# YJxyzxyz/road-vision-system

Hardware: AMD Instinct MI355X
Metric: end-to-end frames/sec @1080p (preproc+YOLOv8n+SORT), 1/2/4/8 MI355X (higher is better)
Workload: dtype bf16

## Files before the change

road-vision-system_amd/csrc/conv.hip:

```cpp
#include <algorithm>
#include <cstdlib>
#include <cstring>
#include "conv.h"
#include "conv_common.h"

namespace rv {

template <int MR, int NR, int WC>
__global__ __launch_bounds__(256, 2) void conv_mfma_kernel(ConvArgs a) {
  constexpr int WP = 4 / WC;
  const int tid = threadIdx.x;
  const int wave = tid >> 6, lane = tid & 63;
  const int col = lane & 15, quad = lane >> 4;
  const int wp = wave % WP, wc = wave / WP;
  const int cout_pad = (a.Cout + 15) & ~15;
  const int cout0 = (blockIdx.y * WC + wc) * (16 * MR);
  const int HWo = a.Ho * a.Wo;
  const int M = a.B * HWo;
  const int pix0 = (blockIdx.x * WP + wp) * (16 * NR);
  if (cout0 >= cout_pad || pix0 >= M) return;

  const int cin_pad = (a.Cin + 31) & ~31;
  const int kspt = cin_pad >> 5;
  const int Kp = a.k * a.k * cin_pad;
// ... 107 lines not shown
          float* o = (float*)outp;
          const float4 pk = make_float4(v[0], v[1], v[2], v[3]);
          if (!up) {
            *(float4*)(o + opix * cs_ + co_) = pk;
          } else {
            for (int dy = 0; dy < 2; ++dy)
              for (int dx = 0; dx < 2; ++dx) {
                const size_t q = ((size_t)(b * 2 * a.Ho + 2 * oy + dy) * (2 * a.Wo) + 2 * ox + dx);
                *(float4*)(o + q * cs_ + co_) = pk;
              }
          }
        } else {
          uint16_t* o = (uint16_t*)outp;
          const uint2 pk = make_uint2(pack_bf16x2(v[0], v[1]), pack_bf16x2(v[2], v[3]));
          if (!up) {
            *(uint2*)(o + opix * cs_ + co_) = pk;
          } else {
            for (int dy = 0; dy < 2; ++dy)
              for (int dx = 0; dx < 2; ++dx) {
                const size_t q = ((size_t)(b * 2 * a.Ho + 2 * oy + dy) * (2 * a.Wo) + 2 * ox + dx);
                *(uint2*)(o + q * cs_ + co_) = pk;
              }
          }
        }
      }
    }
  }
}

template <int MR, int NR, int WC>
static void launch_t(const ConvArgs& a, hipStream_t s) {
  constexpr int WP = 4 / WC;
  const int M = a.B * a.Ho * a.Wo;
  const int T = (a.Cout + 15) / 16;
  dim3 grid(ceil_div(M, 16 * NR * WP), ceil_div(T, MR * WC));
  conv_mfma_kernel<MR, NR, WC><<<grid, 256, 0, s>>>(a);
}

static int try_launch_patch(const ConvArgs& a, hipStream_t s, int* st);

static bool vcat(const ConvArgs& a) { return a.split > 0 || a.in_up; }

int launch_conv(const ConvArgs& a, hipStream_t s) {
  int st = 0;
  if (vcat(a)) {
    const int T = (a.Cout + 15) / 16;
    ConvCfg c{1, 1, 1, 1, 1, 1};
    for (const int mr : {8, 4, 2})
      if (T % mr == 0 && conv_cfg_ok(a, ConvCfg{mr, 1, 1, 1, 1, 1})) {
        c.mr = mr;
        break;
      }
    if (!conv_cfg_ok(a, c)) {
      set_error("virtual concat input (split %d, up %d) needs a bf16 1x1 conv", a.split, a.in_up);
      return RV_EINVAL;
    }
    return launch_conv_cfg(a, c, s);
  }
  if (try_launch_patch(a, s, &st)) return st;
  if (a.ch_w) {
    set_error("chained 1x1 conv (Cout %d, k%d s%d) has no patch-kernel configuration", a.Cout, a.k,
              a.stride);
    return RV_EINVAL;
  }
  if (a.in8) {
    set_error("fp8 conv (Cin %d, Cout %d, k%d s%d) has no patch-kernel configuration", a.Cin,
              a.Cout, a.k, a.stride);
    return RV_EINVAL;
  }
  if (a.g2_cout0 > 0) {
    set_error("grouped conv (Cout %d, split %d) has no patch-kernel configuration", a.Cout,
              a.g2_cout0);
    return RV_EINVAL;
  }
  const int T = (a.Cout + 15) / 16;
  const long M = (long)a.B * a.Ho * a.Wo;
  struct Cand {
    int mr, nr;
  };
  static const Cand cands[] = {{4, 4}, {2, 8}, {4, 2}, {2, 4}, {1, 8}, {4, 1}, {2, 2},
                               {1, 4}, {2, 1}, {1, 2}, {1, 1}};
  int MR = 1, NR = 1;
  for (const Cand& c : cands) {
    if (c.mr > T) continue;
    const int waste = ceil_div(T, c.mr) * c.mr - T;
    if (waste > 1 && c.mr > 1) continue;
    const long waves = (long)ceil_div((int)((M + 16 * c.nr - 1) / (16 * c.nr)), 1) * ceil_div(T, c.mr);
    MR = c.mr;
    NR = c.nr;
    if (waves >= 2048) break;
  }
  const int groups_c = ceil_div(T, MR);
  const int WC = groups_c >= 4 ? 4 : (groups_c >= 2 ? 2 : 1);
#define RV_CONV_WC(mr, nr)                                           \
  if (MR == mr && NR == nr) {                                        \
    if (WC == 4) launch_t<mr, nr, 4>(a, s);                          \
    else if (WC == 2) launch_t<mr, nr, 2>(a, s);                     \
    else launch_t<mr, nr, 1>(a, s);                                  \
    return launch_status("conv_mfma");                               \
  }
  RV_CONV_WC(4, 4) RV_CONV_WC(2, 8) RV_CONV_WC(4, 2) RV_CONV_WC(2, 4) RV_CONV_WC(1, 8)
  RV_CONV_WC(4, 1) RV_CONV_WC(2, 2) RV_CONV_WC(1, 4) RV_CONV_WC(2, 1) RV_CONV_WC(1, 2)
  RV_CONV_WC(1, 1)
#undef RV_CONV_WC
  set_error("no conv variant for MR=%d NR=%d", MR, NR);
  return RV_EINVAL;
}

__device__ __attribute__((aligned(64))) uint4 g_zero16[4];
#ifdef RV_PHASE_PROF
__device__ unsigned long long g_conv_phase[8];
#define RV_PH_T() __builtin_amdgcn_s_memtime()
#endif

struct TileWalk {
  int t0, step, end;
  __device__ __forceinline__ int count() const { return t0 < end ? (end - t0 + step - 1) / step : 0; }
};
__device__ __forceinline__ TileWalk tile_walk(int ntiles) {
  const int gx = gridDim.x, bx = blockIdx.x;
  if ((gx & 7) == 0) {
    const int chunk = (ntiles + 7) >> 3, j = bx & 7;
    return TileWalk{j * chunk + (bx >> 3), gx >> 3, min(ntiles, (j + 1) * chunk)};
  }
  return TileWalk{bx, gx, ntiles};
}
static inline int xcd_grid(int want, int ntiles, bool persist) {
  if (!persist) return ntiles >= 8 ? (ntiles + 7) & ~7 : ntiles;
  const int g = std::min(want, ntiles);
  return g >= 8 ? g & ~7 : g;
}

#ifndef RV_CONV_IN_AUX
#define RV_CONV_IN_AUX 0
#endif
template <int AUX = 0>
__device__ __forceinline__ void dma16(__amdgpu_buffer_rsrc_t r, void* lds, uint32_t voff, int soff) {
  __builtin_amdgcn_raw_ptr_buffer_load_lds(r, (__attribute__((address_space(3))) void*)lds, 16,
                                           (int)voff, soff, 0, AUX);
}

__device__ __forceinline__ float head_sigmoid(float x) {
  return __builtin_amdgcn_rcpf(1.0f + __expf(-x));
}

struct PatchGeo {
  int C, R;
  int G;
  int PH, PW;
  int pinst;
  int tiles_x, tiles_y;
  int p_bytes;
  int fast;
  int stagger;
};

static bool epi_fast(const ConvArgs& a) {
  static const bool off = getenv("RV_EPI_SLOW") != nullptr;
  const double px = (double)a.B * a.Ho * a.Wo;
  return !off && !a.out_f32 && !a.out1 && !a.out0_up && !a.in8 && a.Cout % 16 == 0 && px < (1 << 23) &&
         a.out0_cs < 2048 && px * a.out0_cs * 2 < 2147483647.0 &&
         (!a.res || (a.res_cs < 2048 && px * a.res_cs * 2 < 2147483647.0));
}

template <int MR, int NR>
__device__ __forceinline__ void epilogue_fast(const ConvArgs& a, f32x4 (&acc)[MR][NR], int cout0,
                                              const bool (&pv)[NR], const uint32_t (&opx)[NR],
                                              int quad, const f32x4 (&bias)[MR]) {
  const __amdgpu_buffer_rsrc_t ro = __builtin_amdgcn_make_buffer_rsrc(a.out0, 0, 0x7FFFFFFF, kRsrcFlags);
  const __amdgpu_buffer_rsrc_t rr =
      __builtin_amdgcn_make_buffer_rsrc((void*)a.res, 0, 0x7FFFFFFF, kRsrcFlags);
  const int cq = cout0 + quad * 4;
  constexpr uint32_t kDrop = 0x80000000u;
  auto value = [&](int m, int n, uint32_t vr, uint32_t& lo, uint32_t& hi) {
    float v[4];
#pragma unroll
    for (int i = 0; i < 4; ++i) v[i] = acc[m][n][i] + bias[m][i];
    if (a.act) {
      silu4(v);
    }
    if (a.res) {
      const uint32_t roff = cout0 + m * 16 < a.Cout ? vr + m * 32 : kDrop;
      const uint2 q = __builtin_bit_cast(
          uint2, __builtin_amdgcn_raw_buffer_load_b64(rr, (int)roff, 0, 0));
      v[0] += bf2f(q.x & 0xFFFF);
      v[1] += bf2f(q.x >> 16);
      v[2] += bf2f(q.y & 0xFFFF);
      v[3] += bf2f(q.y >> 16);
    }
    lo = pack_bf16x2(v[0], v[1]);
    hi = pack_bf16x2(v[2], v[3]);
  };
#pragma unroll
  for (int n = 0; n < NR; ++n) {
    if (!pv[n]) continue;
    const uint32_t vo = (__umul24(opx[n], (uint32_t)a.out0_cs) + a.out0_co + cq) * 2;
    const uint32_t vr = a.res ? (__umul24(opx[n], (uint32_t)a.res_cs) + a.res_co + cq) * 2 : 0u;
    const uint32_t vo16 = vo + (16 * (quad & 1) + 8 * (quad >> 1) - 4 * quad) * 2;
#pragma unroll
    for (int m = 0; m + 1 < MR; m += 2) {
      if (cout0 + m * 16 >= a.Cout) continue;
      uint32_t a0, a1, b0, b1;
      value(m, n, vr, a0, a1);
      value(m + 1, n, vr, b0, b1);
      const auto x0 = __builtin_amdgcn_permlane16_swap(a0, b0, false, false);
      const auto x1 = __builtin_amdgcn_permlane16_swap(a1, b1, false, false);
      const bool ok = cout0 + (m + (quad & 1)) * 16 < a.Cout;
      const uint32_t off = ok ? vo16 + m * 32 : kDrop;
      const v4u32 pk = {x0[0], x1[0], x0[1], x1[1]};
      __builtin_amdgcn_raw_buffer_store_b128(pk, ro, (int)off, 0, 0);
    }
    if constexpr (MR & 1) {
      constexpr int m = MR - 1;
      if (cout0 + m * 16 < a.Cout) {
        uint32_t lo, hi;
        value(m, n, vr, lo, hi);
        __builtin_amdgcn_raw_buffer_store_b64(v2u32{lo, hi}, ro, (int)(vo + m * 32), 0, 0);
      }
    }
  }
}

template <int MR, int NR>
struct EpiPend {
  v4u32 pk[MR / 2 > 0 ? MR / 2 : 1][NR];
  uint32_t off[MR / 2 > 0 ? MR / 2 : 1][NR];
  v2u32 pk1[NR];
  uint32_t off1[NR];
};

template <int MR, int NR>
__device__ __forceinline__ void epi_pack(const ConvArgs& a, f32x4 (&acc)[MR][NR], int cout0,
                                         const bool (&pv)[NR], const uint32_t (&opx)[NR], int quad,
                                         const f32x4 (&bias)[MR], EpiPend<MR, NR>& ep) {
  const __amdgpu_buffer_rsrc_t rr =
      __builtin_amdgcn_make_buffer_rsrc((void*)a.res, 0, 0x7FFFFFFF, kRsrcFlags);
  const int cq = cout0 + quad * 4;
  constexpr uint32_t kDrop = 0x80000000u;
  uint2 rq[MR][NR];
  if (a.res) {
#pragma unroll
    for (int n = 0; n < NR; ++n) {
      const uint32_t vr = (__umul24(opx[n], (uint32_t)a.res_cs) + a.res_co + cq) * 2;
#pragma unroll
      for (int m = 0; m < MR; ++m) {
        const uint32_t roff = pv[n] && cout0 + m * 16 < a.Cout ? vr + m * 32 : kDrop;
        rq[m][n] = __builtin_bit_cast(uint2, __builtin_amdgcn_raw_buffer_load_b64(rr, (int)roff, 0, 0));
      }
    }
  }
  auto value = [&](int m, int n, uint32_t vr, uint32_t& lo, uint32_t& hi) {
    (void)vr;
    float v[4];
#pragma unroll
    for (int i = 0; i < 4; ++i) v[i] = acc[m][n][i] + bias[m][i];
    if (a.act) silu4(v);
    if (a.res) {
      const uint2 q = rq[m][n];
      v[0] += bf2f(q.x & 0xFFFF);
      v[1] += bf2f(q.x >> 16);
      v[2] += bf2f(q.y & 0xFFFF);
      v[3] += bf2f(q.y >> 16);
    }
    lo = pack_bf16x2(v[0], v[1]);
    hi = pack_bf16x2(v[2], v[3]);
  };
#pragma unroll
  for (int n = 0; n < NR; ++n) {
    const uint32_t vo = (__umul24(opx[n], (uint32_t)a.out0_cs) + a.out0_co + cq) * 2;
    const uint32_t vr = a.res ? (__umul24(opx[n], (uint32_t)a.res_cs) + a.res_co + cq) * 2 : 0u;
    const uint32_t vo16 = vo + (16 * (quad & 1) + 8 * (quad >> 1) - 4 * quad) * 2;
#pragma unroll
    for (int m = 0; m + 1 < MR; m += 2) {
      uint32_t a0, a1, b0, b1;
      value(m, n, vr, a0, a1);
      value(m + 1, n, vr, b0, b1);
      const auto x0 = __builtin_amdgcn_permlane16_swap(a0, b0, false, false);
      const auto x1 = __builtin_amdgcn_permlane16_swap(a1, b1, false, false);
      const bool ok = pv[n] && cout0 + (m + (quad & 1)) * 16 < a.Cout;
      ep.off[m / 2][n] = ok ? vo16 + m * 32 : kDrop;
      ep.pk[m / 2][n] = v4u32{x0[0], x1[0], x0[1], x1[1]};
    }
    if constexpr (MR & 1) {
      constexpr int m = MR - 1;
      uint32_t lo, hi;
      value(m, n, vr, lo, hi);
      ep.off1[n] = pv[n] && cout0 + m * 16 < a.Cout ? vo + m * 32 : kDrop;
      ep.pk1[n] = v2u32{lo, hi};
    }
  }
}

template <int MR, int NR>
__device__ __forceinline__ void epi_store(const ConvArgs& a, const EpiPend<MR, NR>& ep) {
  const __amdgpu_buffer_rsrc_t ro = __builtin_amdgcn_make_buffer_rsrc(a.out0, 0, 0x7FFFFFFF, kRsrcFlags);
#pragma unroll
  for (int n = 0; n < NR; ++n) {
#pragma unroll
    for (int m = 0; m + 1 < MR; m += 2)
      __builtin_amdgcn_raw_buffer_store_b128(ep.pk[m / 2][n], ro, (int)ep.off[m / 2][n], 0, 0);
    if constexpr (MR & 1) __builtin_amdgcn_raw_buffer_store_b64(ep.pk1[n], ro, (int)ep.off1[n], 0, 0);
  }
}

template <bool F8>
__device__ __forceinline__ int swzq(int i) {
  return F8 ? (i >> 2) & 3 : (i >> 1) & 2;
// ... 186 lines not shown
  bool oin[NR];
#pragma unroll
  for (int n = 0; n < NR; ++n) {
    const int q = wave * (NR * 16) + n * 16 + col;
    orow[n] = q / g.C;
    ocol[n] = q - orow[n] * g.C;
    oin[n] = q < g.R * g.C;
    const int pr = oin[n] ? orow[n] * S : 0, pc = oin[n] ? ocol[n] * S : 0;
#pragma unroll
    for (int kx = 0; kx < K; ++kx) {
      const int sc = patch_scol<S>(pc + kx, g.PW);
      const int lq = F8 ? quad >> 1 : quad;
      if constexpr (F8 && K == 3)
        boff[n][kx] = (pr * g.PW + sc) * 64 + swzq<true>(sc);
      else
        boff[n][kx] = (pr * g.PW + sc) * 64 + ((lq ^ swzq<F8>(sc)) << 4) + (F8 ? (quad & 1) * 8 : 0);
    }
  }
  int aoff[F8 && K == 3 ? MR : 1][2];
  if constexpr (F8 && K == 3) {
#pragma unroll
    for (int m = 0; m < MR; ++m) {
      const int row = m * 16 + col, sw = swzq<true>(row);
      const int base = (row * T2 + (quad >> 1)) * 64;
      aoff[m][0] = base + (((2 * (quad & 1)) ^ sw) << 4);
      aoff[m][1] = base + (((2 * (quad & 1) + 1) ^ sw) << 4);
    }
  }
  float* const bias_lds = (float*)(stages + 2 * stage_bytes);
  f32x4 bias[F8 ? MR : 1], dq[F8 ? MR : 1];
  if constexpr (F8) {
#pragma unroll
    for (int m = 0; m < MR; ++m) {
      const int co = wc0 + m * 16 + quad * 4;
      bias[m] = co < wcout_pad ? *(const f32x4*)(bias_p + co) : f32x4{0.f, 0.f, 0.f, 0.f};
      const f32x4 ws = co < wcout_pad ? *(const f32x4*)(wsc_p + co) : f32x4{0.f, 0.f, 0.f, 0.f};
      dq[m] = ws * a.s_in;
    }
  } else {
    for (int i = tid; i < BC; i += 64 * NW) bias_lds[i] = wc0 + i < wcout_pad ? bias_p[wc0 + i] : 0.f;
  }
  auto bias_tile = [&](f32x4 (&bl)[MR]) {
#pragma unroll
    for (int m = 0; m < MR; ++m) bl[m] = *(const f32x4*)(bias_lds + m * 16 + quad * 4);
  };
  constexpr int CHN = (MR + 1) / 2;
  constexpr int CHF = BC + 4;
  uint8_t* const ch_w_lds = (uint8_t*)(bias_lds + BC);
  float* const ch_b_lds = (float*)(ch_w_lds + (CH ? CHN * BC * 64 : 0));
  uint8_t* const ch_x_lds = (uint8_t*)(ch_b_lds + (CH ? BC : 0)) + wave * (CH ? CHN * NR * 16 * 64 : 0);
  float* const ch_f_lds = (float*)((uint8_t*)(ch_b_lds + (CH ? BC : 0)) + NW * (CH ? CHN * NR * 16 * 64 : 0)) +
                          wave * (CHM == 2 ? NR * 16 * CHF : 0);
  if constexpr (CH) {
    static_assert(!F8 && K == 3, "chained 1x1: bf16 behind a 3x3 conv");
    for (int j = wave; j < CHN * (BC / 16); j += NW) {
      const int c = j / (BC / 16), jr = j - c * (BC / 16);
      const int row = jr * 16 + (lane >> 2);
      const int q = (lane & 3) ^ swzq<false>(row);
      __builtin_amdgcn_global_load_lds((const void*)(a.ch_w + (size_t)row * (CHN * 32) + c * 32 + q * 8),
                                       (void*)(ch_w_lds + c * BC * 64 + jr * 1024), 16, 0, 0);
    }
    for (int i = tid; i < BC; i += 64 * NW) ch_b_lds[i] = a.ch_b[i];
    if constexpr (MR % 2) {
      for (int px = lane; px < NR * 16; px += 64) {
        uint8_t* sl = ch_x_lds + ((CHN - 1) * NR * 16 + px) * 64;
        *(uint4*)(sl + ((2 ^ swzq<false>(px)) << 4)) = make_uint4(0, 0, 0, 0);
        *(uint4*)(sl + ((3 ^ swzq<false>(px)) << 4)) = make_uint4(0, 0, 0, 0);
      }
    }
  }
  uint32_t tailbad = 0;
  int lgeo[MAXP];
#pragma unroll
  for (int it = 0; it < MAXP; ++it) {
    const int L = 64 * (wave + NW * it) + lane;
    const int pix = L / SL, q = L - SL * pix;
    const int py = (int)(((float)pix + 0.5f) * inv_pw);
    const int sc = pix - py * g.PW;
    const int he = (g.PW + 1) >> 1;
    const int px = S == 1 ? sc : (sc < he ? 2 * sc : 2 * (sc - he) + 1);
    const int sq = q ^ swzq<F8>(sc);
    lgeo[it] = (pix < npp ? py : 4095) | (px << 12) | (sq << 24);
    if ((nch - 1) * CC + sq * (16 / EB) >= Cin) tailbad |= 1u << it;
  }
  const bool has_tail = Cin % CC != 0;
  uint32_t voff[MAXP];
  __amdgpu_buffer_rsrc_t img_rsrc;
  const int pix_bytes = a.in_cs * EB;
  auto prep_tile = [&](int ti) {
    const int b = ti / tiles_img;
    const int r = ti - b * tiles_img;
    const int ty = r / g.tiles_x, tx = r - (r / g.tiles_x) * g.tiles_x;
    const int iy0 = ty * g.R * S - pad, ix0 = tx * g.C * S - pad;
    const uint8_t* base = (const uint8_t*)a.in + ((size_t)b * a.Hin * a.Win * a.in_cs + in_co) * EB;
    img_rsrc = __builtin_amdgcn_make_buffer_rsrc((void*)base, 0,
                                                 (a.Hin * a.Win * a.in_cs - in_co) * EB, kRsrcFlags);
#pragma unroll
    for (int it = 0; it < MAXP; ++it) {
      const int gg = lgeo[it];
      const int iy = iy0 + (gg & 4095), ix = ix0 + ((gg >> 12) & 4095);
      const bool ok = (unsigned)iy < (unsigned)a.Hin && (unsigned)ix < (unsigned)a.Win;
      const uint32_t off = __umul24((uint32_t)(__umul24(iy, a.Win) + ix), (uint32_t)pix_bytes) +
                           ((gg >> 24) & 3) * 16;
      const uint32_t m = ok ? 0u : 0xFFFFFFFFu;
      voff[it] = (off & ~m) | (kOOB & m);
    }
  };
  const __amdgpu_buffer_rsrc_t w_rsrc = __builtin_amdgcn_make_buffer_rsrc(
      (void*)(wts + (size_t)wc0 * Kp * EB), 0, (wcout_pad - wc0) * Kp * EB, kRsrcFlags);
  uint32_t wvoff[MAXW];
#pragma unroll
  for (int it = 0; it < MAXW; ++it) {
    const int j = wave + NW * it;
    const int pr = j * 16 + (lane >> 2);
    const int row = pr / T2, tap = pr - (pr / T2) * T2;
    const int q = (lane & 3) ^ swzq<F8>(row);
    wvoff[it] = wc0 + row < wcout_pad ? (uint32_t)((row * Kp + tap * cin_pad) * EB + q * 16) : kOOB;
  }
  auto dma_weights = [&](int c, uint8_t* Wl) {
#pragma unroll
    for (int it = 0; it < MAXW; ++it) {
      const int j = wave + NW * it;
      if (j < WJ) dma16(w_rsrc, Wl + j * 1024, wvoff[it], c * 64);
    }
  };
  auto stage = [&](int grp, int buf) {
    for (int gi = 0; gi < G; ++gi) {
      const int c = grp * G + gi;
      if (c >= nch) break;
      uint8_t* P = stages + buf * stage_bytes + gi * chunk_bytes;
      const bool tail = has_tail && c == nch - 1;
#ifdef RV_DMA_SELECT_ALWAYS
      if (true) {
#else
      if (tail) {
#endif
#pragma unroll
        for (int it = 0; it < MAXP; ++it) {
          const int j = wave + NW * it;
          if (j < g.pinst)
            dma16<RV_CONV_IN_AUX>(img_rsrc, P + j * 1024,
                                  tail && ((tailbad >> it) & 1) ? kOOB : voff[it], c * 64);
        }
      } else {
#pragma unroll
        for (int it = 0; it < MAXP; ++it) {
          const int j = wave + NW * it;
          if (j < g.pinst) dma16<RV_CONV_IN_AUX>(img_rsrc, P + j * 1024, voff[it], c * 64);
        }
      }
      if constexpr (!RESW) dma_weights(c, P + g.p_bytes);
    }
  };
  f32x4 acc[MR][NR];
  auto compute = [&](int grp, int buf) {
    for (int gi = 0; gi < G; ++gi) {
      const int c = grp * G + gi;
      if (c >= nch) break;
      const uint8_t* P = stages + buf * stage_bytes + gi * chunk_bytes;
      const uint8_t* Wl = RESW ? smem + c * W_BYTES : P + g.p_bytes;
      if constexpr (F8 && K == 3) {
        const int rowb = g.PW * PB;
#pragma unroll
        for (int t = 0; t < 9; t += 2) {
          const bool odd = t + 1 >= 9;
          const int ky0 = t / 3, kx0 = t % 3;
          const int ky1 = odd ? ky0 : (t + 1) / 3, kx1 = odd ? kx0 : (t + 1) % 3;
          const bool hi = (quad >> 1) != 0;
          i32x8 A[MR], Bv[NR];
#pragma unroll
          for (int m = 0; m < MR; ++m) {
            const uint4 lo = *(const uint4*)(Wl + aoff[m][0] + t * 64);
            const uint4 up = *(const uint4*)(Wl + aoff[m][1] + t * 64);
            A[m] = i32x8{(int)lo.x, (int)lo.y, (int)lo.z, (int)lo.w,
                         (int)up.x, (int)up.y, (int)up.z, (int)up.w};
            if (odd && hi) A[m] = i32x8{0, 0, 0, 0, 0, 0, 0, 0};
          }
#pragma unroll
          for (int n = 0; n < NR; ++n) {
            const int v = hi ? boff[n][kx1] + ky1 * rowb : boff[n][kx0] + ky0 * rowb;
            const int sw = v & 3, base = v & ~63;
            const uint4 lo = *(const uint4*)(P + base + (((2 * (quad & 1)) ^ sw) << 4));
            const uint4 up = *(const uint4*)(P + base + (((2 * (quad & 1) + 1) ^ sw) << 4));
            Bv[n] = i32x8{(int)lo.x, (int)lo.y, (int)lo.z, (int)lo.w,
                          (int)up.x, (int)up.y, (int)up.z, (int)up.w};
          }
#pragma unroll
          for (int m = 0; m < MR; ++m)
#pragma unroll
            for (int n = 0; n < NR; ++n)
              acc[m][n] = __builtin_amdgcn_mfma_scale_f32_16x16x128_f8f6f4(
                  A[m], Bv[n], acc[m][n], 0, 0, 0, 127, 0, 127);
        }
        continue;
      }
      if constexpr (!F8 && MR * NR < 16) {
        bf16x8 Af[2][MR], Bq[2][NR];
        auto ld = [&](int tap, int sl) {
          const int ky = tap / K, kx = tap - (tap / K) * K;
#pragma unroll
          for (int m = 0; m < MR; ++m) {
            const int row = m * 16 + col;
            Af[sl][m] = __builtin_bit_cast(
                bf16x8, *(const uint4*)(Wl + (row * T2 + tap) * 64 + ((quad ^ swzq<false>(row)) << 4)));
          }
#pragma unroll
          for (int n = 0; n < NR; ++n)
            Bq[sl][n] = __builtin_bit_cast(bf16x8, *(const uint4*)(P + ky * g.PW * PB + boff[n][kx]));
        };
        ld(0, 0);
#pragma unroll
        for (int t = 0; t < T2; ++t) {
          if (t + 1 < T2) ld(t + 1, (t + 1) & 1);
          __builtin_amdgcn_sched_barrier(0);
#pragma unroll
          for (int m = 0; m < MR; ++m)
#pragma unroll
            for (int n = 0; n < NR; ++n)
              acc[m][n] = __builtin_amdgcn_mfma_f32_16x16x32_bf16(Af[t & 1][m], Bq[t & 1][n],
                                                                  acc[m][n], 0, 0, 0);
          __builtin_amdgcn_sched_barrier(0);
        }
        continue;
      }
#pragma unroll(F8 || MR * NR >= 16 ? 1 : K)
      for (int ky = 0; ky < K; ++ky) {
        const uint8_t* Prow = P + ky * g.PW * PB;
#pragma unroll
        for (int kx = 0; kx < K; ++kx) {
          const int tap = ky * K + kx;
          if constexpr (F8) {
#pragma unroll
            for (int hh = 0; hh < 2; ++hh) {
              long A[MR], Bf[NR];
#pragma unroll
              for (int m = 0; m < MR; ++m) {
                const int row = m * 16 + col;
                A[m] = *(const long*)(Wl + (((row * T2 + tap) * 64 +
                                             (((quad >> 1) ^ swzq<true>(row)) << 4) + (quad & 1) * 8) ^
                                            (hh << 5)));
              }
#pragma unroll
              for (int n = 0; n < NR; ++n) Bf[n] = *(const long*)(Prow + (boff[n][kx] ^ (hh << 5)));
              __builtin_amdgcn_sched_barrier(0);
#pragma unroll
              for (int m = 0; m < MR; ++m)
#pragma unroll
                for (int n = 0; n < NR; ++n)
                  acc[m][n] = __builtin_amdgcn_mfma_f32_16x16x32_fp8_fp8(A[m], Bf[n], acc[m][n], 0, 0, 0);
            }
          } else {
            bf16x8 A[MR], Bf[NR];
#pragma unroll
            for (int m = 0; m < MR; ++m) {
              const int row = m * 16 + col;
              A[m] = __builtin_bit_cast(
                  bf16x8, *(const uint4*)(Wl + (row * T2 + tap) * 64 + ((quad ^ swzq<false>(row)) << 4)));
            }
#pragma unroll
            for (int n = 0; n < NR; ++n)
              Bf[n] = __builtin_bit_cast(bf16x8, *(const uint4*)(Prow + boff[n][kx]));
            __builtin_amdgcn_sched_barrier(0);
#pragma unroll
            for (int m = 0; m < MR; ++m)
#pragma unroll
              for (int n = 0; n < NR; ++n)
                acc[m][n] = __builtin_amdgcn_mfma_f32_16x16x32_bf16(A[m], Bf[n], acc[m][n], 0, 0, 0);
          }
        }
      }
    }
  };

  if (nsteps == 0) return;
#ifdef RV_PHASE_PROF
  unsigned long long ph[5] = {0, 0, 0, 0, 0}, t_ph = RV_PH_T();
#define RV_PH(i)                             \
  {                                          \
    const unsigned long long t_ = RV_PH_T(); \
    ph[i] += t_ - t_ph;                      \
    t_ph = t_;                               \
  }
#else
#define RV_PH(i)
#endif
  int ti = walk.t0;
  int grp = 0;
  constexpr bool kStagger = NW == 8 && !(MR == 5 && NR == 2) && !(MR == 2 && NR == 4);
  const bool late = kStagger && g.stagger && wave >= 4;
  bool pend = false;
  int ptile = 0;
  constexpr bool kDefer = !F8 && !CH && MR * NR <= 10;
  auto chain_tile = [&](const bool (&pv)[NR], const uint32_t (&opx)[NR]) {
    if constexpr (CH) {
      f32x4 bl[MR];
      bias_tile(bl);
      if constexpr (MR % 2) {
#pragma unroll
        for (int n = 0; n < NR; ++n) {
          const int px = n * 16 + col;
#pragma unroll
          for (int m = 0; m < MR; ++m) {
            float v[4];
#pragma unroll
            for (int i = 0; i < 4; ++i) v[i] = acc[m][n][i] + bl[m][i];
            if (a.act) silu4(v);
            const int qq = 2 * (m & 1) + (quad >> 1);
            *(v2u32*)(ch_x_lds + ((m / 2) * NR * 16 + px) * 64 + ((qq ^ swzq<false>(px)) << 4) +
                      (quad & 1) * 8) = v2u32{pack_bf16x2(v[0], v[1]), pack_bf16x2(v[2], v[3])};
          }
        }
      } else {
#pragma unroll
      for (int n = 0; n < NR; ++n) {
        const int px = n * 16 + col;
#pragma unroll
        for (int m = 0; m < MR; m += 2) {
          uint32_t v0[2], v1[2];
#pragma unroll
          for (int h = 0; h < 2; ++h) {
            float v[4];
#pragma unroll
            for (int i = 0; i < 4; ++i) v[i] = acc[m + h][n][i] + bl[m + h][i];
            if (a.act) silu4(v);
            v0[h] = pack_bf16x2(v[0], v[1]);
            v1[h] = pack_bf16x2(v[2], v[3]);
          }
          const auto x0 = __builtin_amdgcn_permlane16_swap(v0[0], v0[1], false, false);
          const auto x1 = __builtin_amdgcn_permlane16_swap(v1[0], v1[1], false, false);
          const int qq = 2 * (quad & 1) + (quad >> 1);
          *(v4u32*)(ch_x_lds + ((m / 2) * NR * 16 + px) * 64 + ((qq ^ swzq<false>(px)) << 4)) =
              v4u32{x0[0], x1[0], x0[1], x1[1]};
        }
      }
      }
      f32x4 acc2[MR][NR];
#pragma unroll
      for (int m = 0; m < MR; ++m)
#pragma unroll
        for (int n = 0; n < NR; ++n) acc2[m][n] = f32x4{0.f, 0.f, 0.f, 0.f};
#pragma unroll
      for (int c = 0; c < CHN; ++c) {
        bf16x8 A2[MR], B2[NR];
#pragma unroll
        for (int m = 0; m < MR; ++m) {
          const int row = m * 16 + col;
          A2[m] = __builtin_bit_cast(
              bf16x8, *(const uint4*)(ch_w_lds + c * BC * 64 + row * 64 + ((quad ^ swzq<false>(row)) << 4)));
        }
#pragma unroll
        for (int n = 0; n < NR; ++n) {
          const int px = n * 16 + col;
          B2[n] = __builtin_bit_cast(
              bf16x8, *(const uint4*)(ch_x_lds + (c * NR * 16 + px) * 64 + ((quad ^ swzq<false>(px)) << 4)));
        }
#pragma unroll
        for (int m = 0; m < MR; ++m)
#pragma unroll
          for (int n = 0; n < NR; ++n)
            acc2[m][n] = __builtin_amdgcn_mfma_f32_16x16x32_bf16(A2[m], B2[n], acc2[m][n], 0, 0, 0);
      }
      f32x4 bl2[MR];
#pragma unroll
      for (int m = 0; m < MR; ++m) bl2[m] = *(const f32x4*)(ch_b_lds + m * 16 + quad * 4);
      if constexpr (CHM == 1) {
        ConvArgs a2 = a;
        a2.act = 1;
        a2.res = nullptr;
        epilogue_fast<MR, NR>(a2, acc2, 0, pv, opx, quad, bl2);
      } else if constexpr (CHM == 2) {
        static_assert(MR == 4, "box branch: 4 sides of 16 bins");
#pragma unroll
        for (int n = 0; n < NR; ++n)
#pragma unroll
          for (int m = 0; m < MR; ++m)
            *(f32x4*)(ch_f_lds + (n * 16 + col) * CHF + m * 16 + quad * 4) = acc2[m][n] + bl2[m];
        const int pxl = lane >> 2, part = lane & 3;
#pragma unroll
        for (int n = 0; n < NR; ++n) {
          const float* row = ch_f_lds + (n * 16 + pxl) * CHF + part * 16;
          float v[16];
#pragma unroll
          for (int i = 0; i < 16; i += 4) {
            const f32x4 q4 = *(const f32x4*)(row + i);
            v[i] = q4[0];
            v[i + 1] = q4[1];
            v[i + 2] = q4[2];
            v[i + 3] = q4[3];
          }
          float mx = -INFINITY;
#pragma unroll
          for (int i = 0; i < 16; ++i) mx = fmaxf(mx, v[i]);
          float sum = 0.f;
#pragma unroll
          for (int i = 0; i < 16; ++i) {
            v[i] = __expf(v[i] - mx);
            sum += v[i];
          }
          const float rs = __builtin_amdgcn_rcpf(sum);
          float e = 0.f;
#pragma unroll
          for (int i = 0; i < 16; ++i) e += (float)i * (v[i] * rs);
          const int base = lane & ~3;
          const float d0 = __shfl(e, base), d1 = __shfl(e, base + 1), d2 = __shfl(e, base + 2),
                      d3 = __shfl(e, base + 3);
          const uint32_t o = (uint32_t)__shfl((int)opx[n], pxl);
          const bool ok = __shfl((int)pv[n], pxl) != 0;
          if (part == 0 && ok) *(f32x4*)((float*)a.out0 + (size_t)o * 4) = f32x4{d0, d1, d2, d3};
        }
      } else {
#pragma unroll
        for (int n = 0; n < NR; ++n) {
          float best = -1.f;
          int bc = 0;
#pragma unroll
          for (int m = 0; m < MR; ++m) {
            const int co = m * 16 + quad * 4;
            const f32x4 v = acc2[m][n] + bl2[m];
#pragma unroll
            for (int i = 0; i < 4; ++i) {
              const float sg = head_sigmoid(v[i]);
              if (co + i < a.Cout && sg > best) {
                best = sg;
                bc = co + i;
              }
            }
          }
#pragma unroll
          for (int off = 16; off < 64; off <<= 1) {
            const float ob = __shfl_xor(best, off);
            const int oc = __shfl_xor(bc, off);
            if (ob > best || (ob == best && oc < bc)) {
              best = ob;
              bc = oc;
            }
          }
          if (quad == 0 && pv[n])
            *(v2u32*)((float*)a.out0 + (size_t)opx[n] * 2) =
                v2u32{__float_as_uint(best), (uint32_t)bc};
        }
      }
    }
  };
  auto finish = [&](int tile, EpiPend<MR, NR>& ep, bool pk) {
    const int b = tile / tiles_img;
    const int r = tile - b * tiles_img;
    const int ty = r / g.tiles_x, tx = r - (r / g.tiles_x) * g.tiles_x;
    bool pv[NR];
    int pb[NR], py[NR], px[NR];
#pragma unroll
    for (int n = 0; n < NR; ++n) {
      pb[n] = b;
      py[n] = ty * g.R + orow[n];
      px[n] = tx * g.C + ocol[n];
      pv[n] = oin[n] && py[n] < a.Ho && px[n] < a.Wo;
    }
#ifdef RV_EPI_SKIP
    if (a.Cout == 12345) {
      float t = 0.f;
#pragma unroll
      for (int m = 0; m < MR; ++m)
#pragma unroll
        for (int n = 0; n < NR; ++n) t += acc[m][n][0] + acc[m][n][3];
      ((float*)a.out0)[tid] = t;
    }
    if (true) {
    } else
#endif
    if constexpr (F8) {
      epilogue8<MR, NR>(a, acc, cout0, pv, pb, py, px, quad, bias, dq);
    } else if constexpr (CH) {
      uint32_t opx[NR];
#pragma unroll
      for (int n = 0; n < NR; ++n) opx[n] = (uint32_t)((b * a.Ho + py[n]) * a.Wo + px[n]);
      chain_tile(pv, opx);
    } else if (g.fast) {
      uint32_t opx[NR];
#pragma unroll
      for (int n = 0; n < NR; ++n) opx[n] = __umul24((uint32_t)(b * a.Ho + py[n]), (uint32_t)a.Wo) + px[n];
      f32x4 bl[MR];
      bias_tile(bl);
      if constexpr (kDefer) {
        if (pk)
          epi_pack<MR, NR>(a, acc, cout0, pv, opx, quad, bl, ep);
        else
          epilogue_fast<MR, NR>(a, acc, cout0, pv, opx, quad, bl);
      } else {
        epilogue_fast<MR, NR>(a, acc, cout0, pv, opx, quad, bl);
      }
    } else {
      f32x4 bl[MR];
      bias_tile(bl);
      epilogue<MR, NR>(a, acc, cout0, pv, pb, py, px, quad, bl);
    }
  };
  if constexpr (RESW)
    for (int c = 0; c < nch; ++c) dma_weights(c, smem + c * W_BYTES);
  prep_tile(ti);
  stage(0, 0);
  __syncthreads();
  RV_PH(0);
  for (int s = 0; s < nsteps; ++s) {
    EpiPend<MR, NR> ep;
    if (kStagger && pend) {
      finish(ptile, ep, false);
      pend = false;
    }
    if (grp == 0) {
#pragma unroll
      for (int m = 0; m < MR; ++m)
#pragma unroll
        for (int n = 0; n < NR; ++n) acc[m][n] = f32x4{0.f, 0.f, 0.f, 0.f};
    }
    const bool last = grp + 1 == ngrp;
    if (s + 1 < nsteps) {
      if (last) prep_tile(ti + walk.step);
      stage(last ? 0 : grp + 1, (s + 1) & 1);
    }
    RV_PH(1);
    compute(grp, s & 1);
    RV_PH(2);
    if (last) {
      if (late) {
        pend = true;
        ptile = ti;
      } else {
        finish(ti, ep, true);
      }
      ti += walk.step;
      grp = 0;
      RV_PH(3);
    } else {
      ++grp;
    }
    __syncthreads();
    if constexpr (kDefer) {
      if (last && g.fast && !late) epi_store<MR, NR>(a, ep);
    }
    RV_PH(4);
  }
  if (kStagger && pend) {
    EpiPend<MR, NR> ep;
    finish(ptile, ep, false);
  }
#ifdef RV_PHASE_PROF
  if (lane == 0) {
#pragma unroll
    for (int i = 0; i < 5; ++i) atomicAdd(&g_conv_phase[i], ph[i]);
    atomicAdd(&g_conv_phase[5], (unsigned long long)nsteps);
    atomicAdd(&g_conv_phase[6], 1ull);
  }
#endif
#undef RV_PH
}


template <int MR, int NR>
__global__ __launch_bounds__(256, 2) void conv1x1_direct_kernel(ConvArgs a, int fast) {
  extern __shared__ __attribute__((aligned(16))) uint8_t smem[];
  constexpr int BC = 16 * MR;
  constexpr int W_BYTES = BC * 64;
  constexpr int WJ = BC / 16;
  constexpr int MAXW = (WJ + 3) / 4;
  const int tid = threadIdx.x;
  const int wave = tid >> 6, lane = tid & 63;
  const int col = lane & 15, quad = lane >> 4;
  const int cout0 = blockIdx.y * BC;
  const int wcout_pad = (a.Cout + 15) & ~15;
  const int cin_pad = (a.Cin + 31) & ~31;
  const int nch = cin_pad >> 5;
  const int HW = a.Ho * a.Wo;
  const int npix = a.B * HW;
  const int ntiles = (npix + 64 * NR - 1) / (64 * NR);
  for (int c = 0; c < nch; ++c) {
#pragma unroll
    for (int it = 0; it < MAXW; ++it) {
      const int j = wave + 4 * it;
      if (j < WJ) {
        const int row = j * 16 + (lane >> 2);
        const int q = (lane & 3) ^ swzq<false>(row);
        const int co = cout0 + row;
        const void* src = co < wcout_pad ? (const void*)(a.w + (size_t)co * cin_pad + q * 8 + c * 32)
                                         : (const void*)g_zero16;
        __builtin_amdgcn_global_load_lds(src, (void*)(smem + c * W_BYTES + j * 1024), 16, 0, 0);
      }
    }
  }
  __syncthreads();
  f32x4 bias[MR];
#pragma unroll
  for (int m = 0; m < MR; ++m) {
    const int co = cout0 + m * 16 + quad * 4;
    bias[m] = co < wcout_pad ? *(const f32x4*)(a.bias + co) : f32x4{0.f, 0.f, 0.f, 0.f};
  }
  int aoff[MR];
#pragma unroll
  for (int m = 0; m < MR; ++m) {
    const int row = m * 16 + col;
    aoff[m] = row * 64 + ((quad ^ swzq<false>(row)) << 4);
  }
  const bool need_geo = a.in_up || !fast;
  const TileWalk walk = tile_walk(ntiles);
  struct Geo {
    const bf16_t* src[NR];
    const bf16_t* src2[NR];
    bool pv[NR];
    int pb[NR], py[NR], px[NR];
  };
  auto geo = [&](int t, Geo& G) {
#pragma unroll
    for (int n = 0; n < NR; ++n) {
      const int p = t * 64 * NR + wave * 16 * NR + n * 16 + col;
      G.pv[n] = t < walk.end && p < npix;
      const int pp = G.pv[n] ? p : 0;
      G.pb[n] = G.py[n] = G.px[n] = 0;
      if (need_geo) {
        G.pb[n] = pp / HW;
        const int r = pp - G.pb[n] * HW;
        G.py[n] = r / a.Wo;
        G.px[n] = r - G.py[n] * a.Wo;
      }
      const size_t ps = a.in_up ? ((size_t)G.pb[n] * (a.Ho >> 1) + (G.py[n] >> 1)) * (a.Wo >> 1) +
                                      (G.px[n] >> 1)
                                : (size_t)pp;
      G.src[n] = a.in + ps * a.in_cs + a.in_co + quad * 8;
      G.src2[n] = a.in2 + (size_t)pp * a.in2_cs + a.in2_co + quad * 8 - a.split;
    }
  };
  auto load = [&](const Geo& G, int c, uint4 (&B)[NR]) {
    const bool kin = c * 32 + quad * 8 < a.Cin;
    const bool second = a.split > 0 && c * 32 >= a.split;
#pragma unroll
    for (int n = 0; n < NR; ++n)
      B[n] = *(const uint4*)((G.pv[n] && kin) ? (const void*)((second ? G.src2[n] : G.src[n]) + c * 32)
                                              : (const void*)g_zero16);
  };
  auto mma = [&](int c, const uint4 (&B)[NR], f32x4 (&acc)[MR][NR]) {
    const uint8_t* Wl = smem + c * W_BYTES;
    bf16x8 A[MR];
#pragma unroll
    for (int m = 0; m < MR; ++m) A[m] = __builtin_bit_cast(bf16x8, *(const uint4*)(Wl + aoff[m]));
    __builtin_amdgcn_sched_barrier(0);
#pragma unroll
    for (int m = 0; m < MR; ++m)
#pragma unroll
      for (int n = 0; n < NR; ++n)
        acc[m][n] = __builtin_amdgcn_mfma_f32_16x16x32_bf16(A[m], __builtin_bit_cast(bf16x8, B[n]),
                                                            acc[m][n], 0, 0, 0);
  };
  auto finish = [&](int t, const Geo& G, f32x4 (&acc)[MR][NR]) {
    if (fast) {
      uint32_t opx[NR];
#pragma unroll
      for (int n = 0; n < NR; ++n) opx[n] = (uint32_t)(t * 64 * NR + wave * 16 * NR + n * 16 + col);
      epilogue_fast<MR, NR>(a, acc, cout0, G.pv, opx, quad, bias);
    } else {
      epilogue<MR, NR>(a, acc, cout0, G.pv, G.pb, G.py, G.px, quad, bias);
    }
  };
  const int P = (nch + 1) & ~1;
  uint4 B0[NR], B1[NR];
  Geo G0, G1;
  int t = walk.t0;
  geo(t, G0);
  geo(t + walk.step, G1);
  load(G0, 0, B0);
  load(G0, 1, B1);
  for (; t < walk.end; t += walk.step) {
    f32x4 acc[MR][NR];
#pragma unroll
    for (int m = 0; m < MR; ++m)
#pragma unroll
      for (int n = 0; n < NR; ++n) acc[m][n] = f32x4{0.f, 0.f, 0.f, 0.f};
    for (int c = 0; c < P - 2; c += 2) {
      mma(c, B0, acc);
      __builtin_amdgcn_sched_barrier(0);
      load(G0, c + 2, B0);
      __builtin_amdgcn_sched_barrier(0);
      mma(c + 1, B1, acc);
      __builtin_amdgcn_sched_barrier(0);
      load(G0, c + 3, B1);
      __builtin_amdgcn_sched_barrier(0);
    }
    mma(P - 2, B0, acc);
    __builtin_amdgcn_sched_barrier(0);
    load(G1, 0, B0);
    __builtin_amdgcn_sched_barrier(0);
    if (P - 1 < nch) mma(P - 1, B1, acc);
    __builtin_amdgcn_sched_barrier(0);
    load(G1, 1, B1);
    __builtin_amdgcn_sched_barrier(0);
    finish(t, G0, acc);
    G0 = G1;
    geo(t + 2 * walk.step, G1);
  }
}

static int conv_nch(const ConvArgs& a) {
  int cin = a.Cin;
  if (a.g2_cout0 > 0 && a.g2_Cin > cin) cin = a.g2_Cin;
  const int cc = a.in8 ? 64 : 32;
  return (cin + cc - 1) / cc;
}

static bool patch_geo(const ConvArgs& a, const ConvCfg& c, PatchGeo& g, size_t& smem) {
  if (!((a.k == 1 || a.k == 3) && (a.stride == 1 || a.stride == 2) && a.pad == a.k / 2)) return false;
  if ((size_t)a.Hin * a.Win >= (1u << 24) || (size_t)a.in_cs * 2 >= (1u << 24)) return false;
  const int NR = c.nr, MR = c.mr;
  const int NW = c.kind == 2 ? 8 : 4;
  const int P = 16 * NR * NW;
  struct TileKey {
    int wo, ho, s, k, p, c;
  };
  static thread_local TileKey memo[64];
  static thread_local int memo_n = 0, memo_w = 0;
  int C = 0;
  for (int i = 0; i < memo_n && !C; ++i)
    if (memo[i].wo == a.Wo && memo[i].ho == a.Ho && memo[i].s == a.stride && memo[i].k == a.k &&
        memo[i].p == P)
      C = memo[i].c;
  if (!C) {
    long best = -1;
    for (int c = std::min(a.Wo, P); c >= std::min(16, a.Wo); --c) {
      const int r = P / c;
      const long cost = (long)ceil_div(a.Wo, c) * ceil_div(a.Ho, r) * ((r - 1) * a.stride + a.k) *
                        ((c - 1) * a.stride + a.k);
      if (best < 0 || cost < best) {
        best = cost;
        C = c;
      }
    }
    memo[memo_w++ & 63] = TileKey{a.Wo, a.Ho, a.stride, a.k, P, C};
    memo_n = std::min(memo_n + 1, 64);
  }
  g.C = C;
  g.R = P / C;
  if (g.R < 1) return false;
  g.PH = (g.R - 1) * a.stride + a.k;
  g.PW = (g.C - 1) * a.stride + a.k;
  g.pinst = ceil_div(g.PH * g.PW * 4, 64);
  g.p_bytes = g.pinst * 1024;
  g.tiles_x = ceil_div(a.Wo, g.C);
  g.tiles_y = ceil_div(a.Ho, g.R);
  const int nch = conv_nch(a);
  g.G = std::max(1, std::min(c.G, nch));
  g.fast = epi_fast(a) ? 1 : 0;
  static const int stagger = getenv("RV_STAGGER") ? atoi(getenv("RV_STAGGER")) : 0;
  g.stagger = stagger;
  const int maxit = (a.stride == 2 ? 6 : 2) * NR + 2;
  if (ceil_div(g.pinst, NW) > maxit) return false;
  const size_t wb = (size_t)16 * MR * a.k * a.k * 64;
  smem = (c.resw ? nch * wb : 0) + 2 * (size_t)g.G * (g.p_bytes + (c.resw ? 0 : wb)) +
         (a.in8 ? 0 : (size_t)16 * MR * 4);
  if (a.ch_w) {
    const size_t chn = (MR + 1) / 2;
    smem += chn * 16 * MR * 64 + (size_t)16 * MR * 4 + (size_t)NW * chn * NR * 16 * 64 +
            (a.ch_mode == 2 ? (size_t)NW * NR * 16 * (16 * MR + 4) * 4 : 0);
  }
  return smem <= 160 * 1024;
}

static int num_cus() {
  static int n = 0;
  if (!n) {
    int dev = 0;
    hipDeviceProp_t p;
    if (hipGetDevice(&dev) == hipSuccess && hipGetDeviceProperties(&p, dev) == hipSuccess)
      n = p.multiProcessorCount;
    else
      n = 256;
    (void)hipGetLastError();
  }
  return n;
}

template <int MR, int NR, int K, int S, bool RESW, bool F8 = false, int NW = 4, int CHM = 0>
static int launch_patch_t(const ConvArgs& a, const PatchGeo& g, size_t smem, int persist,
                          hipStream_t s) {
  static bool attr = false;
  auto fn = conv_patch_kernel<MR, NR, K, S, RESW, F8, NW, CHM>;
  if (!attr) {
    hipError_t e = hipFuncSetAttribute((const void*)fn, hipFuncAttributeMaxDynamicSharedMemorySize,
                                       160 * 1024);
    if (e != hipSuccess) {
      (void)hipGetLastError();
      set_error("hipFuncSetAttribute: %s", hipGetErrorString(e));
      return -(int)e;
    }
    attr = true;
  }
  static size_t occ_smem[16] = {0};
  static int occ_val[16] = {0};
  int occ = 0;
  for (int i = 0; i < 16; ++i)
    if (occ_smem[i] == smem) occ = occ_val[i];
  if (!occ) {
    if (hipOccupancyMaxActiveBlocksPerMultiprocessor(&occ, fn, 64 * NW, smem) != hipSuccess || occ < 1)
      occ = 1;
    (void)hipGetLastError();
    for (int i = 0; i < 16; ++i)
      if (occ_smem[i] == 0) {
        occ_smem[i] = smem;
        occ_val[i] = occ;
        break;
      }
  }
  const int T = (a.Cout + 15) / 16;
  const int ytiles = ceil_div(T, MR);
  const int ntiles = a.B * g.tiles_x * g.tiles_y;
  const int gx = xcd_grid(std::max(1, num_cus() * occ / ytiles), ntiles, persist != 0);
  dim3 grid(gx, ytiles);
  fn<<<grid, 64 * NW, smem, s>>>(a, g);
  return launch_status("conv_patch");
}

static size_t direct_smem(const ConvArgs& a, int MR) {
  return (size_t)((a.Cin + 31) / 32) * 16 * MR * 64;
}

template <int MR, int NR>
static int launch_direct_t(const ConvArgs& a, int persist, hipStream_t s) {
  static bool attr = false;
  auto fn = conv1x1_direct_kernel<MR, NR>;
  if (!attr) {
    hipError_t e = hipFuncSetAttribute((const void*)fn, hipFuncAttributeMaxDynamicSharedMemorySize,
                                       160 * 1024);
    if (e != hipSuccess) {
      (void)hipGetLastError();
      set_error("hipFuncSetAttribute: %s", hipGetErrorString(e));
      return -(int)e;
    }
    attr = true;
  }
  const size_t smem = direct_smem(a, MR);
  static size_t occ_smem[16] = {0};
  static int occ_val[16] = {0};
  int occ = 0;
  for (int i = 0; i < 16; ++i)
    if (occ_smem[i] == smem) occ = occ_val[i];
  if (!occ) {
    if (hipOccupancyMaxActiveBlocksPerMultiprocessor(&occ, fn, 256, smem) != hipSuccess || occ < 1)
      occ = 1;
    (void)hipGetLastError();
    for (int i = 0; i < 16; ++i)
      if (occ_smem[i] == 0) {
        occ_smem[i] = smem;
        occ_val[i] = occ;
        break;
      }
  }
  const int ytiles = ceil_div((a.Cout + 15) / 16, MR);
  const int ntiles = ceil_div(a.B * a.Ho * a.Wo, 64 * NR);
  const int gx = xcd_grid(std::max(1, num_cus() * occ / ytiles), ntiles, persist != 0);
  fn<<<dim3(gx, ytiles), 256, smem, s>>>(a, epi_fast(a) ? 1 : 0);
  return launch_status("conv1x1_direct");
}

static bool direct_ok(const ConvArgs& a, const ConvCfg& c) {
  const int T = (a.Cout + 15) / 16;
  const bool vcat_ok = (a.split == 0 && !a.in_up) ||
                       (a.split % 32 == 0 && a.split <= a.Cin && (!a.in_up || (a.Ho % 2 == 0 && a.Wo % 2 == 0)) &&
                        (a.split == a.Cin || (a.in2 && a.in2_cs % 8 == 0 && a.in2_co % 8 == 0)));
  return a.k == 1 && a.stride == 1 && a.pad == 0 && a.g2_cout0 <= 0 && a.Hin == a.Ho &&
         a.Win == a.Wo && (c.mr <= T || c.mr == 1) && a.in_cs % 8 == 0 && a.in_co % 8 == 0 &&
         !a.in8 && vcat_ok && direct_smem(a, c.mr) <= 160 * 1024;
}


template <int MR, int NR>
constexpr bool patch_s2_ok() {
  return NR <= 2 && MR * NR <= 8;
}

constexpr bool patch_spills(int MR, int NR, int K, int S, bool RESW) {
  return !RESW && K == 3 && ((S == 1 && MR * NR > 16) || (S == 2 && MR * NR >= 8));
}

template <int MR, int NR>
constexpr bool tile8_built() {
  return (MR == 1 || MR == 2 || MR == 4) && (NR == 1 || NR == 2 || NR == 4);
}
constexpr bool patch_spills8(int MR, int NR, int K, int S, bool RESW) {
  return K == 3 && (MR * NR >= 16 || (S == 1 && MR == 2 && NR == 4) ||
                    (S == 2 && !RESW && MR == 1 && NR == 2));
}

template <int MR, int NR, int CHM>
constexpr bool ch_built() {
  return NR <= 2 && ((CHM <= 2 && MR == 4) || (CHM == 3 && MR == 5));
}
static bool ch_tile_ok(int mr, int nr, int mode) {
  return nr <= 2 && ((mode <= 2 && mr == 4) || (mode == 3 && mr == 5));
}
template <int MR, int NR, bool RESW, int NW>
static int launch_patch_ch(const ConvArgs& a, const PatchGeo& g, size_t smem, int persist,
                           hipStream_t s) {
  if constexpr (ch_built<MR, NR, 1>()) {
    if (a.ch_mode == 1 && a.k == 3 && a.stride == 2)
      return launch_patch_t<MR, NR, 3, 2, RESW, false, NW, 1>(a, g, smem, persist, s);
    if (a.ch_mode == 1 && a.k == 3 && a.stride == 1)
      return launch_patch_t<MR, NR, 3, 1, RESW, false, NW, 1>(a, g, smem, persist, s);
// ... 896 lines not shown
```

Baseline: 44460.

## Interleave next-tile prep with MFMA compute and drop staggered epilogue path

Moves the per-tile index/offset preparation (prep_tile) for the tile after next out of the serial step loop and into the compute loop, right after the first tap's MFMAs, so its scalar/ALU work overlaps matrix math. This applies to non-F8 configurations except two MR/NR shapes. It also removes the env-gated staggered-epilogue mechanism and adds a phase-profile slot. The prep now runs one tile further ahead, which may raise register pressure and costs the unused stagger option.

```diff
diff --git a/road-vision-system_amd/csrc/conv.hip b/road-vision-system_amd/csrc/conv.hip
--- a/road-vision-system_amd/csrc/conv.hip
+++ b/road-vision-system_amd/csrc/conv.hip
@@ -283,7 +283,6 @@
   int tiles_x, tiles_y;
   int p_bytes;
   int fast;
-  int stagger;
 };
 
 static bool epi_fast(const ConvArgs& a) {
@@ -776,11 +775,14 @@
       if constexpr (!RESW) dma_weights(c, P + g.p_bytes);
     }
   };
+  int ti = 0;
   f32x4 acc[MR][NR];
-  auto compute = [&](int grp, int buf) {
+  constexpr bool kPrepAhead = !F8 && !(MR == 5 && NR == 2) && !(MR == 2 && NR == 4);
+  auto compute = [&](int grp, int buf, bool prep, int ptile) {
     for (int gi = 0; gi < G; ++gi) {
       const int c = grp * G + gi;
       if (c >= nch) break;
+      const bool prep_now = kPrepAhead && prep && gi == 0;
       const uint8_t* P = stages + buf * stage_bytes + gi * chunk_bytes;
       const uint8_t* Wl = RESW ? smem + c * W_BYTES : P + g.p_bytes;
       if constexpr (F8 && K == 3) {
@@ -844,6 +846,12 @@
               acc[m][n] = __builtin_amdgcn_mfma_f32_16x16x32_bf16(Af[t & 1][m], Bq[t & 1][n],
                                                                   acc[m][n], 0, 0, 0);
           __builtin_amdgcn_sched_barrier(0);
+          if constexpr (kPrepAhead) {
+            if (t == 0) {
+              if (prep_now) prep_tile(ptile);
+              __builtin_amdgcn_sched_barrier(0);
+            }
+          }
         }
         continue;
       }
@@ -890,6 +898,13 @@
 #pragma unroll
               for (int n = 0; n < NR; ++n)
                 acc[m][n] = __builtin_amdgcn_mfma_f32_16x16x32_bf16(A[m], Bf[n], acc[m][n], 0, 0, 0);
+            if constexpr (kPrepAhead) {
+              if (kx == 0) {
+                __builtin_amdgcn_sched_barrier(0);
+                if (prep_now && ky == 0) prep_tile(ptile);
+                __builtin_amdgcn_sched_barrier(0);
+              }
+            }
           }
         }
       }
@@ -898,7 +913,7 @@
 
   if (nsteps == 0) return;
 #ifdef RV_PHASE_PROF
-  unsigned long long ph[5] = {0, 0, 0, 0, 0}, t_ph = RV_PH_T();
+  unsigned long long ph[6] = {0, 0, 0, 0, 0, 0}, t_ph = RV_PH_T();
 #define RV_PH(i)                             \
   {                                          \
     const unsigned long long t_ = RV_PH_T(); \
@@ -908,12 +923,8 @@
 #else
 #define RV_PH(i)
 #endif
-  int ti = walk.t0;
+  ti = walk.t0;
   int grp = 0;
-  constexpr bool kStagger = NW == 8 && !(MR == 5 && NR == 2) && !(MR == 2 && NR == 4);
-  const bool late = kStagger && g.stagger && wave >= 4;
-  bool pend = false;
-  int ptile = 0;
   constexpr bool kDefer = !F8 && !CH && MR * NR <= 10;
   auto chain_tile = [&](const bool (&pv)[NR], const uint32_t (&opx)[NR]) {
     if constexpr (CH) {
@@ -1122,35 +1133,32 @@
     for (int c = 0; c < nch; ++c) dma_weights(c, smem + c * W_BYTES);
   prep_tile(ti);
   stage(0, 0);
+  if constexpr (kPrepAhead) {
+    if (ngrp == 1 && nsteps > 1) prep_tile(ti + walk.step);
+  }
   __syncthreads();
   RV_PH(0);
   for (int s = 0; s < nsteps; ++s) {
     EpiPend<MR, NR> ep;
-    if (kStagger && pend) {
-      finish(ptile, ep, false);
-      pend = false;
-    }
     if (grp == 0) {
 #pragma unroll
       for (int m = 0; m < MR; ++m)
 #pragma unroll
         for (int n = 0; n < NR; ++n) acc[m][n] = f32x4{0.f, 0.f, 0.f, 0.f};
     }
-    const bool last = grp + 1 == ngrp;
-    if (s + 1 < nsteps) {
-      if (last) prep_tile(ti + walk.step);
-      stage(last ? 0 : grp + 1, (s + 1) & 1);
-    }
+    const bool last = grp + 1 == ngrp, more = s + 1 < nsteps;
+    if constexpr (!kPrepAhead) {
+      if (more && last) prep_tile(ti + walk.step);
+    }
+    RV_PH(5);
+    if (more) stage(last ? 0 : grp + 1, (s + 1) & 1);
     RV_PH(1);
-    compute(grp, s & 1);
+    const bool one = ngrp == 1;
+    compute(grp, s & 1, s + 2 < nsteps && (one || grp + 2 == ngrp),
+            one ? ti + 2 * walk.step : ti + walk.step);
     RV_PH(2);
     if (last) {
-      if (late) {
-        pend = true;
-        ptile = ti;
-      } else {
-        finish(ti, ep, true);
-      }
+      finish(ti, ep, true);
       ti += walk.step;
       grp = 0;
       RV_PH(3);
@@ -1159,13 +1167,9 @@
     }
     __syncthreads();
     if constexpr (kDefer) {
-      if (last && g.fast && !late) epi_store<MR, NR>(a, ep);
+      if (last && g.fast) epi_store<MR, NR>(a, ep);
     }
     RV_PH(4);
-  }
-  if (kStagger && pend) {
-    EpiPend<MR, NR> ep;
-    finish(ptile, ep, false);
   }
 #ifdef RV_PHASE_PROF
   if (lane == 0) {
@@ -1173,6 +1177,7 @@
     for (int i = 0; i < 5; ++i) atomicAdd(&g_conv_phase[i], ph[i]);
     atomicAdd(&g_conv_phase[5], (unsigned long long)nsteps);
     atomicAdd(&g_conv_phase[6], 1ull);
+    atomicAdd(&g_conv_phase[7], ph[5]);
   }
 #endif
 #undef RV_PH
@@ -1369,8 +1374,6 @@
   const int nch = conv_nch(a);
   g.G = std::max(1, std::min(c.G, nch));
   g.fast = epi_fast(a) ? 1 : 0;
-  static const int stagger = getenv("RV_STAGGER") ? atoi(getenv("RV_STAGGER")) : 0;
-  g.stagger = stagger;
   const int maxit = (a.stride == 2 ? 6 : 2) * NR + 2;
   if (ceil_div(g.pinst, NW) > maxit) return false;
   const size_t wb = (size_t)16 * MR * a.k * a.k * 64;
```

After: 44670 (median of 2 runs). Within noise of the previous version (+0.5%).
